# lucasjinreal/yolov7_d2

Hardware: AMD Instinct MI355X
Metric: images/sec training, YOLOX-s 640x640 bs=16/GPU (higher is better)
Workload: dtype bf16; 1 GPU; YOLOX-s CSPDarknet+PAFPN 640x640 bs=16/GPU: fwd + SimOTA loss + bwd + grad all-reduce + SGD(momentum) step, uint8 image batch + labels resident in HBM; global_batch=16, parallelism=dp1, hipgraph=True

## Files before the change

yolov7_d2_amd/csrc/conv3x3_ws.h:

```cpp
#pragma once
#include "common.h"
#include "conv_bn.h"

#define W3_MAX_JOBS 8
#define W3_TW 16
template <int S, int TH>
struct W3Geo {
  static constexpr int HH = S == 1 ? TH + 2 : 2 * TH + 1;
  static constexpr int HW = S == 1 ? W3_TW + 2 : 2 * W3_TW + 1;
  static constexpr int HPIX = HH * HW;
  static constexpr int HROWS = (HPIX + 63) / 64 * 64;
  static constexpr int tap(int dy, int dx) { return S == 1 ? dy * HW + dx : dy * HW + (dx & 1) * (W3_TW + 1) + (dx >> 1); }
};

struct W3Job {
  const __bf16* x;
  const u32x4* w;
  __bf16* y;
  double* stats;
  int ldx, ldy, N, H, W, tilesY, tilesX, ntiles;
  int blk0, nblk;
  int wld, nslots, sld, pad_;
  int tw[9];
  int inH;
  CBnFwd bn;
  int inW, xfw;
  const BnXf* xf;
};
struct W3K {
  int njobs, dbg;
  W3Job j[W3_MAX_JOBS];
};
struct W3Launch {
  int K, MODE, grid, lds, S, XF;
  W3K k;
};

#define W3_VMCNT(n) asm volatile("s_waitcnt vmcnt(%0)" ::"n"(n) : "memory")

static __device__ uint4 g_w3_zero_page[4];
static __device__ __attribute__((aligned(256))) unsigned g_w3_bar[MI_BN_BAR_WORDS];

__device__ __forceinline__ void w3_glds16(const void* g, unsigned lds_off) {
  asm volatile("s_mov_b32 m0, %1\n\ts_nop 0\n\tglobal_load_lds_dwordx4 %0, off" ::"v"(g), "s"(lds_off) : "memory");
}

template <int K, int WM, int WN, int G, int MODE, int S = 1, int TH = 8, int XF = 0>
__global__ __launch_bounds__(WM* WN * 64, (K == 128 || (S == 2 && K == 64)) ? 1 : 2) void w3_kernel(const W3K p) {
  static_assert(!XF || MODE == 1, "the input transform comes with the forward (statistics) mode");
  constexpr int NW = WM * WN, KC8 = K / 8, KS = K / 16;
  using Geo = W3Geo<S, TH>;
  constexpr int W3_TH = TH, W3_HW = Geo::HW, W3_HPIX = Geo::HPIX, W3_HROWS = Geo::HROWS;
  static_assert(WN * G * 32 == W3_TH * W3_TW, "pixel tile");
  constexpr int PLANE = W3_HROWS * 16;
  constexpr int NQ = (W3_HROWS / 64) * KC8;
  constexpr int D = NQ / NW;
  static_assert(NQ % NW == 0 && D >= 1, "DMA split");
  constexpr int XB = KC8 * PLANE;
  static_assert((KC8 - 1) * PLANE + Geo::tap(2, 2) * 16 < 65536, "ds_read immediate");
  constexpr int NS = 9 * KS, NTS = NS / 3;
  constexpr int NST = 2 * G;
  constexpr int DST = 2 * (D - 1) < NTS ? 2 : 1, SST = 2 * NST + NST / 2 <= NTS ? 2 : 1;
  static_assert(DST * (D - 1) < NTS && SST * NST + (MODE == 2 ? NST / 2 : 0) <= NTS, "the memory operations of a tile fit its main loop");

  extern __shared__ __attribute__((aligned(16))) char smem[];
  const unsigned lds0 = (unsigned)(uintptr_t)(__attribute__((address_space(3))) char*)smem;
  const int tid = threadIdx.x, lane = tid & 63;
  const int wave = __builtin_amdgcn_readfirstlane(tid >> 6);
  const int wm = wave / WN, wn = wave % WN;
  const int l31 = lane & 31, h = lane >> 5;

  int ji = 0;
  while (ji + 1 < p.njobs && (int)blockIdx.x >= p.j[ji + 1].blk0) ++ji;
  ji = __builtin_amdgcn_readfirstlane(ji);
  const W3Job& jb = p.j[ji];
  const int b = (int)blockIdx.x - jb.blk0, nb = jb.nblk;
  const int nt = (jb.ntiles - b + nb - 1) / nb;
  constexpr bool STATS = MODE == 1 || MODE == 3;
  unsigned gen0 = 0;
  if constexpr (MODE == 3) {
    const int nblk = (int)gridDim.x;
    if (tid == 0)
      gen0 = __hip_atomic_load(bn_bar_gen(g_w3_bar, (int)blockIdx.x % (nblk < BN_BAR_G ? nblk : BN_BAR_G)), __ATOMIC_RELAXED, __HIP_MEMORY_SCOPE_AGENT);
  }
  const int H = jb.H, Wd = jb.W, tilesX = jb.tilesX, tpi = jb.tilesY * jb.tilesX;
  const int inH = S == 1 ? jb.H : jb.inH, inW = S == 1 ? jb.W : jb.inW;
  const int ldxb = jb.ldx * 2, ldyb = jb.ldy * 2;
  const char* const xbase = (const char*)jb.x;
  char* const ybase = (char*)jb.y;
  const char* zpage = (const char*)g_w3_zero_page;
  asm volatile("" : "+s"(zpage));
  float* const s_sc = (float*)(smem + 2 * (K / 8) * Geo::HROWS * 16 + 256 * 32 * 4);
  float* const s_sh = s_sc + K;
  int xf_act = 0, xf_ldab = 0;
  char* xf_a = nullptr;
  if constexpr (XF) {
    const BnXf* const xf = jb.xf;
    bnx_tables(xf, s_sc, s_sh, NW * 64, jb.xfw != 0 && b == 0);
    xf_act = xf->bn.act;
    xf_ldab = xf->bn.lda * 2;
    xf_a = jb.xfw ? (char*)xf->bn.a : nullptr;
  }

  bf16x8 a[9][KS];
  {
    const u32x4* wb = jb.w + wm * 32 + l31;
#pragma unroll
    for (int t = 0; t < 9; ++t) {
      const int slab = jb.tw[t] * KC8;
#pragma unroll
      for (int ks = 0; ks < KS; ++ks) a[t][ks] = __builtin_bit_cast(bf16x8, wb[(size_t)(slab + ks * 2 + h) * jb.wld]);
    }
  }

  struct Org { int img, ty0, tx0; };
  auto tile_origin = [&](int i) {
    const int t = b + i * nb;
// ... 245 lines not shown
    }
  }
  if constexpr (MODE == 3) {
    int* const s_gave_up = (int*)(smem + 16384);
    bn_grid_barrier(g_w3_bar, gen0, (int)blockIdx.x, (int)gridDim.x, s_gave_up);
    const float poison = *s_gave_up ? __builtin_nanf("") : 0.f;
    const CBnFwd& bn = jb.bn;
    float scl, shl;
    cbn_finalize(bn, jb.stats + (wm * 32 + l31) * 2, jb.sld, jb.nslots, wm * 32 + l31, b == 0 && wn == 0 && h == 0, poison, scl, shl);
    float sc[2][8], sh[2][8];
#pragma unroll
    for (int pr = 0; pr < 2; ++pr)
#pragma unroll
      for (int e = 0; e < 8; ++e) {
        sc[pr][e] = __shfl(scl, pr * 16 + h * 8 + e, 64);
        sh[pr][e] = __shfl(shl, pr * 16 + h * 8 + e, 64);
      }
    const int act = bn.act;
    const bool has_res = bn.res != nullptr;
    const size_t ldab = (size_t)bn.lda * 2, ldrb = (size_t)bn.ldres * 2;
    char* const abase = (char*)bn.a + wm * 64 + h * 16;
    const char* const rbase = (const char*)bn.res + wm * 64 + h * 16;
    for (int i = 0; i < nt; ++i) {
      const Org o = tile_origin(i);
      u32x4 v[NST], r[NST];
      size_t pixi[G];
      bool ok[G];
#pragma unroll
      for (int g = 0; g < G; ++g) {
        const int py = o.ty0 + (wn * G + g) * 2 + lg, px = o.tx0 + lidx;
        ok[g] = (py < H) & (px < Wd);
        pixi[g] = ((size_t)o.img * H + py) * Wd + px;
#pragma unroll
        for (int pr = 0; pr < 2; ++pr) {
          v[g * 2 + pr] = r[g * 2 + pr] = u32x4{0u, 0u, 0u, 0u};
          if (ok[g]) {
            v[g * 2 + pr] = *(const u32x4*)(ybase + pixi[g] * (size_t)ldyb + wm * 64 + h * 16 + pr * 32);
            if (has_res) r[g * 2 + pr] = *(const u32x4*)(rbase + pixi[g] * ldrb + pr * 32);
          }
        }
      }
#pragma unroll
      for (int g = 0; g < G; ++g)
#pragma unroll
        for (int pr = 0; pr < 2; ++pr)
          if (ok[g]) *(u32x4*)(abase + pixi[g] * ldab + pr * 32) = cbn_apply8(v[g * 2 + pr], sc[pr], sh[pr], act, has_res, r[g * 2 + pr]);
    }
  }
}

template <int K, int WM, int WN, int G, int MODE, int S = 1, int TH = 8, int XF = 0>
static int w3_launch_one(const W3Launch& l, hipStream_t s) {
  auto fn = w3_kernel<K, WM, WN, G, MODE, S, TH, XF>;
  static bool attr_done = false;
  if (!attr_done) {
    hipFuncSetAttribute((const void*)fn, hipFuncAttributeMaxDynamicSharedMemorySize, 160 * 1024);
    attr_done = true;
  }
  hipLaunchKernelGGL(fn, dim3((unsigned)l.grid), dim3(WM * WN * 64), (size_t)l.lds, s, l.k);
  MI_CHECK_LAUNCH("conv3x3_ws");
  return MI_OK;
}
constexpr int w3_tile_h(int S, int K) { return S == 1 ? 8 : (K == 128 ? 2 : 4); }
constexpr int w3_block_cout(int S, int K) { return S == 1 ? K : (K == 32 ? 64 : 128); }
template <int MODE, int XF = 0>
static int w3_launch_mode(const W3Launch& l, hipStream_t s) {
  if (l.S == 2) {
    if constexpr (MODE == 1 || MODE == 0) {
      switch (l.K) {
        case 128: return w3_launch_one<128, 4, 1, 1, MODE, 2, 2, XF>(l, s);
        case 64: return w3_launch_one<64, 4, 1, 2, MODE, 2, 4, XF>(l, s);
        case 32: return w3_launch_one<32, 2, 2, 1, MODE, 2, 4, XF>(l, s);
      }
    }
    MI_FAIL(MI_EINVAL, "conv3x3_ws: stride 2 with K %d / mode %d", l.K, MODE);
  }
  switch (l.K) {
    case 128: return w3_launch_one<128, 4, 1, 4, MODE, 1, 8, XF>(l, s);
    case 64: return w3_launch_one<64, 2, 2, 2, MODE, 1, 8, XF>(l, s);
    case 32: return w3_launch_one<32, 1, 4, 1, MODE, 1, 8, XF>(l, s);
  }
  MI_FAIL(MI_EINVAL, "conv3x3_ws: K %d", l.K);
}
```

yolov7_d2_amd/csrc/conv3x3_ws.hip:

```cpp
#include <stdlib.h>
#include <string.h>
#include "common.h"
#include "conv3x3_ws.h"

int w3_launch_mode0(const W3Launch& l, hipStream_t s);
int w3_launch_mode1(const W3Launch& l, hipStream_t s);
int w3_launch_mode1x(const W3Launch& l, hipStream_t s);
int w3_launch_mode2(const W3Launch& l, hipStream_t s);
int w3_launch_mode3(const W3Launch& l, hipStream_t s);
int w3_mode3_blocks_per_cu(int K, int lds);
int w3_bar_status(unsigned* flag);
bool cbn_from_job(const mi_conv_desc& d, const mi_bn_job& j, CBnFwd* o);

static int w3_cus() {
  static int cus = 0;
  if (!cus) {
    int dev = 0;
    hipDeviceProp_t pr;
    if (hipGetDevice(&dev) == hipSuccess && hipGetDeviceProperties(&pr, dev) == hipSuccess) cus = pr.multiProcessorCount;
    if (cus <= 0) cus = 256;
  }
  return cus;
}

static bool w3_desc_ok(const mi_conv_desc* d, int* tw) {
  const int K = d->K8 * 8;
  if (d->ntaps != 9 || (d->in_stride != 1 && d->in_stride != 2) || d->out_stride != 1 || d->out_oy || d->out_ox) return false;
  if (d->gridH != d->outH || d->gridW != d->outW) return false;
  if (d->flags & ~MI_CONV_ACCUM) return false;
  if (d->bias) return false;
  if (!(K == 32 || K == 64 || K == 128) || d->Cout != d->CoutPad) return false;
  if (d->in_stride == 1) {
    if (d->outH != d->H || d->outW != d->W || d->Cout != K) return false;
  } else {
    const char* s2 = getenv("MI_CONV_WS_S2");
    if ((s2 && atoi(s2) == 0) || (d->flags & MI_CONV_ACCUM)) return false;
    if (d->outH != (d->H - 1) / 2 + 1 || d->outW != (d->W - 1) / 2 + 1) return false;
    const int bc = w3_block_cout(2, K);
    if (d->Cout % bc || d->Cout / bc > W3_MAX_JOBS) return false;
  }
  if (d->ldx % 8 || d->ldy % 8 || ((uintptr_t)d->x & 15) || ((uintptr_t)d->y & 15) || ((uintptr_t)d->w & 15)) return false;
  if (d->y_nstride && (long long)d->y_nstride != (long long)d->outH * d->outW * d->ldy) return false;
  if ((long long)d->H * d->W * d->ldx * 2 >= (1LL << 31)) return false;
  if ((d->flags & MI_CONV_ACCUM) && d->stats_acc) return false;
  int seen = 0;
  for (int t = 0; t < 9; ++t) {
    const int dy = d->tap_dy[t], dx = d->tap_dx[t];
    if (dy < -1 || dy > 1 || dx < -1 || dx > 1) return false;
    const int pos = (dy + 1) * 3 + dx + 1;
    if (seen & (1 << pos)) return false;
    seen |= 1 << pos;
    tw[pos] = d->tap_w[t];
  }
  return seen == 0x1ff;
}

static bool w3_fill(const mi_conv_desc* ds, int n, W3Launch* l, const mi_bn_job* bn = nullptr) {
  if (n < 1 || n > W3_MAX_JOBS) return false;
  memset(l, 0, sizeof(*l));
  const int K = ds[0].K8 * 8, S = ds[0].in_stride;
  if (bn && ((ds[0].flags & MI_CONV_ACCUM) || !ds[0].stats_acc || S != 1)) return false;
  const int mode = (ds[0].flags & MI_CONV_ACCUM) ? 2 : (ds[0].stats_acc ? (bn ? 3 : 1) : 0);
  const bool xf = ds[0].xf != nullptr;
  if (xf && mode != 1) return false;
  const int TH = w3_tile_h(S, K);
  const int hrows = ((S == 1 ? (TH + 2) * (W3_TW + 2) : (2 * TH + 1) * (2 * W3_TW + 1)) + 63) / 64 * 64;
  const int lds = 2 * (K / 8) * hrows * 16 + ((mode == 1 || mode == 3) ? 256 * 32 * 4 : 0) + (xf ? 2 * K * 4 : 0);
  long long total = 0;
  int nj = 0;
  for (int j = 0; j < n; ++j) {
    const mi_conv_desc& d = ds[j];
    int tw[9];
    if (!w3_desc_ok(&d, tw) || d.K8 * 8 != K || d.in_stride != S) return false;
    if ((d.flags & MI_CONV_ACCUM) != (ds[0].flags & MI_CONV_ACCUM) || (d.stats_acc != nullptr) != (ds[0].stats_acc != nullptr)) return false;
    if ((d.xf != nullptr) != xf || (xf && (d.xf_C != K || ((uintptr_t)d.xf & 7)))) return false;
    const int bc = w3_block_cout(S, K);
    for (int c0 = 0; c0 < d.Cout; c0 += bc, ++nj) {
      if (nj >= W3_MAX_JOBS) return false;
      W3Job& jb = l->k.j[nj];
      memcpy(jb.tw, tw, sizeof(tw));
      jb.x = (const __bf16*)d.x; jb.w = (const u32x4*)d.w + c0; jb.y = (__bf16*)d.y + c0;
      jb.stats = d.stats_acc ? d.stats_acc + (size_t)c0 * 2 : nullptr;
      jb.ldx = d.ldx; jb.ldy = d.ldy; jb.N = d.N; jb.H = d.outH; jb.W = d.outW; jb.inH = d.H; jb.inW = d.W;
      jb.tilesY = mi_cdiv(d.outH, TH); jb.tilesX = mi_cdiv(d.outW, W3_TW);
      jb.ntiles = d.N * jb.tilesY * jb.tilesX;
      jb.wld = d.CoutPad;
      jb.nslots = (d.stats_slots >= 1 && d.stats_slots <= MI_BN_SLOTS) ? d.stats_slots : MI_BN_SLOTS;
      jb.sld = d.CoutPad * 2;
      total += jb.ntiles;
      if (bn && !cbn_from_job(d, bn[j], &jb.bn)) return false;
      jb.xf = (const BnXf*)d.xf;
      jb.xfw = (xf && d.xf_write && c0 == 0) ? 1 : 0;
    }
  }
  n = nj;
  static const int ovr = getenv("MI_W3_PERCU") ? atoi(getenv("MI_W3_PERCU")) : 0;
  int per_cu = ovr > 0 ? ovr : (K == 128 ? 1 : (K == 64 ? 2 : 4));
  if (S == 2 && ovr <= 0) per_cu = (160 * 1024) / lds >= 2 && K != 128 ? 2 : 1;
  if (mode == 3) {
    static int occ[3] = {-1, -1, -1};
    int& o = occ[K == 128 ? 0 : (K == 64 ? 1 : 2)];
    if (o < 0) o = w3_mode3_blocks_per_cu(K, lds);
    if (o < 1) return false;
    if (per_cu > o) per_cu = o;
  }
  long long cap = (long long)w3_cus() * per_cu;
  if (cap > total) cap = total;
  int used = 0;
  for (int j = 0; j < n; ++j) {
    W3Job& jb = l->k.j[j];
    long long nb = (cap * jb.ntiles) / total;
    if (nb < 1) nb = 1;
    if (nb > jb.ntiles) nb = jb.ntiles;
    jb.nblk = (int)nb;
    used += jb.nblk;
  }
  while (used < cap) {
    int best = -1;
    double br = 0;
    for (int j = 0; j < n; ++j) {
      const W3Job& jb = l->k.j[j];
      const double r = (double)jb.ntiles / jb.nblk;
      if (jb.nblk < jb.ntiles && r > br) { br = r; best = j; }
    }
    if (best < 0) break;
    l->k.j[best].nblk++;
    used++;
  }
  int blk = 0;
  for (int j = 0; j < n; ++j) {
    l->k.j[j].blk0 = blk;
    blk += l->k.j[j].nblk;
  }
  l->k.njobs = n;
  l->k.dbg = (getenv("MI_DEBUG_NOATOM") ? atoi(getenv("MI_DEBUG_NOATOM")) & 1 : 0) | (getenv("MI_W3_DBG") ? atoi(getenv("MI_W3_DBG")) & 6 : 0);
  l->K = K;
  l->S = S;
  l->MODE = mode;
  l->XF = xf ? 1 : 0;
  l->grid = blk;
  l->lds = lds;
  return true;
}

static int w3_run(const W3Launch& l, hipStream_t s) {
  switch (l.MODE) {
    case 0: return w3_launch_mode0(l, s);
    case 1: return l.XF ? w3_launch_mode1x(l, s) : w3_launch_mode1(l, s);
    case 3: return w3_launch_mode3(l, s);
    default: return w3_launch_mode2(l, s);
  }
}

static bool w3_enabled() {
  const char* e = getenv("MI_CONV_WS");
  return !e || atoi(e) != 0;
}

bool w3_try_launch(const mi_conv_desc* ds, int n, hipStream_t s, int* rc) {
  if (!w3_enabled()) return false;
  W3Launch l;
  if (!w3_fill(ds, n, &l)) return false;
  *rc = w3_run(l, s);
  return true;
}
bool w3_try_plan(const mi_conv_desc* ds, int n, W3Launch* l) { return w3_enabled() && w3_fill(ds, n, l); }
bool w3_try_plan_bn(const mi_conv_desc* ds, const mi_bn_job* bn, int n, W3Launch* l) { return w3_enabled() && w3_fill(ds, n, l, bn); }
int w3_barrier_status(unsigned* flag) { return w3_bar_status(flag); }
int w3_run_planned(const W3Launch* l, hipStream_t s) { return w3_run(*l, s); }

extern "C" int mi_conv3x3_ws(const mi_conv_desc* descs, int n, mi_stream_t st) {
  MI_REQUIRE(descs && n >= 1, "conv3x3_ws: null");
  W3Launch l;
  MI_REQUIRE(w3_fill(descs, n, &l),
             "conv3x3_ws: needs 1..%d bf16 3x3 stride-1 convs with K == Cout in {32, 64, 128} (all the same K), no bias, "
             "all plain / all with stats_acc / all MI_CONV_ACCUM", W3_MAX_JOBS);
  return w3_run(l, (hipStream_t)st);
}
```

yolov7_d2_amd/csrc/conv_igemm.hip:

```cpp
#include <string.h>
#include <string.h>
#include "common.h"
#include "conv_igemm_kernel.h"
#include "conv1x1_stream.h"

bool c1s_try_launch(const mi_conv_desc* ds, int n, hipStream_t s, int* rc);
bool c1s_try_plan(const mi_conv_desc* ds, int n, C1Launch* l);
int c1s_run_planned(const C1Launch* l, hipStream_t s);
bool c1s_try_plan_bn(const mi_conv_desc* ds, const mi_bn_job* bn, int n, C1Launch* l);
int c1s_barrier_status(unsigned* flag);
static_assert(sizeof(C1Launch) <= sizeof(((mi_conv_group*)0)->priv), "mi_conv_group.priv holds the stream launch record");
#include "conv3x3_ws.h"
bool w3_try_launch(const mi_conv_desc* ds, int n, hipStream_t s, int* rc);
bool w3_try_plan(const mi_conv_desc* ds, int n, W3Launch* l);
int w3_run_planned(const W3Launch* l, hipStream_t s);
bool w3_try_plan_bn(const mi_conv_desc* ds, const mi_bn_job* bn, int n, W3Launch* l);
int w3_barrier_status(unsigned* flag);
static_assert(sizeof(W3Launch) <= sizeof(((mi_conv_group*)0)->priv), "mi_conv_group.priv holds the 3x3 launch record");

#define MI_DECL_KC(KCv)                                                                      \
  int conv_launch_kc##KCv(const ConvK& k, int BN, int TPIX, size_t lds, hipStream_t s);       \
  int conv_group_launch_kc##KCv(const mi_conv_group* m, const ConvK* jobs, const int* starts, hipStream_t s);
MI_DECL_KC(16) MI_DECL_KC(32) MI_DECL_KC(64) MI_DECL_KC(128)
#undef MI_DECL_KC

static void choose_tile(int TPIX, int gridH, int gridW, int* TH, int* TW) {
  const int cands[] = {gridW, 64, 32, 16, 8, 4};
  long best = -1;
  int bh = 8, bw = 16;
  for (int c : cands) {
    if (c <= 0 || c > TPIX) continue;
    int tw = c;
    int th = TPIX / tw;
    if (th > gridH) th = gridH;
    if (th < 1) th = 1;
    long tiles = (long)mi_cdiv(gridH, th) * mi_cdiv(gridW, tw);
    long halo = (long)(th + 2) * (tw + 2);
    long score = tiles * 100000 + halo;
    if (best < 0 || score < best) {
      best = score;
      bh = th;
      bw = tw;
    }
  }
  *TH = bh;
  *TW = bw;
}

struct ConvCfg {
  int KC, BN, TPIX, TPS;
};

#ifdef MI_CONV_TIMELINE
static long long* g_conv_tl = nullptr;
extern "C" void mi_debug_conv_timeline(long long* dev_buf) { g_conv_tl = dev_buf; }
#endif
static int conv_fill(const mi_conv_desc* d, ConvK* k, ConvCfg* c, size_t* ldsBytes) {
  MI_REQUIRE(d->x && d->w && d->y, "conv: null pointer");
  MI_REQUIRE(d->ntaps >= 1 && d->ntaps <= MI_MAX_TAPS, "conv: ntaps %d", d->ntaps);
  MI_REQUIRE(d->K8 >= 2 && (d->K8 % 2) == 0, "conv: K8 %d must be even", d->K8);
  MI_REQUIRE(d->CoutPad % 32 == 0 && d->Cout <= d->CoutPad && d->Cout > 0, "conv: Cout %d pad %d",
             d->Cout, d->CoutPad);
  MI_REQUIRE(d->ldx % 8 == 0 && ((uintptr_t)d->x % 16) == 0, "conv: x must be 16B aligned (ldx %d)", d->ldx);
  MI_REQUIRE(d->in_stride == 1 || d->in_stride == 2, "conv: in_stride");
  MI_REQUIRE(d->out_stride == 1 || d->out_stride == 2, "conv: out_stride");
  MI_REQUIRE((long long)d->H * d->W * d->ldx < (1LL << 30), "conv: image plane too large for 32-bit offsets");
  if (!(d->flags & MI_CONV_OUT_F32))
    MI_REQUIRE((d->Cout % 4 != 0) || (d->ldy % 4 == 0 && ((uintptr_t)d->y % 8) == 0),
               "conv: bf16 y needs 8B alignment (ldy %d)", d->ldy);
  k->x = (const __bf16*)d->x;
  k->w = (const u32x4*)d->w;
  k->y = d->y;
  k->bias = d->bias;
  k->stats = d->stats_acc;
  k->nslots = (d->stats_slots >= 1 && d->stats_slots <= MI_BN_SLOTS) ? d->stats_slots : MI_BN_SLOTS;
  k->ynstride = d->y_nstride > 0 ? (long long)d->y_nstride : (long long)d->outH * d->outW * d->ldy;
  k->ldx = d->ldx; k->ldy = d->ldy; k->N = d->N; k->H = d->H; k->W = d->W;
  k->outH = d->outH; k->outW = d->outW; k->gridH = d->gridH; k->gridW = d->gridW;
  k->is = d->in_stride; k->os = d->out_stride; k->ooy = d->out_oy; k->oox = d->out_ox;
  k->K8 = d->K8; k->Cout = d->Cout; k->CoutPad = d->CoutPad; k->ntaps = d->ntaps;
  int dymin = 1 << 30, dymax = -(1 << 30), dxmin = 1 << 30, dxmax = -(1 << 30);
  for (int t = 0; t < d->ntaps; ++t) {
    k->tw[t] = d->tap_w[t];
    if (d->tap_dy[t] < dymin) dymin = d->tap_dy[t];
    if (d->tap_dy[t] > dymax) dymax = d->tap_dy[t];
    if (d->tap_dx[t] < dxmin) dxmin = d->tap_dx[t];
    if (d->tap_dx[t] > dxmax) dxmax = d->tap_dx[t];
  }
  k->flags = d->flags;
  {
    static const int noatom = getenv("MI_DEBUG_NOATOM") ? atoi(getenv("MI_DEBUG_NOATOM")) : 0;
    if (noatom) k->flags |= 1024;
  }
  MI_REQUIRE(!(d->flags & MI_CONV_RELU) || !((d->flags & (MI_CONV_ACCUM | MI_CONV_BNBWD | MI_CONV_OUT_F32 | MI_CONV_RELUMASK | MI_CONV_ADDRELU)) || d->stats_acc),
             "conv: MI_CONV_RELU is a plain forward epilogue (bf16 output, no accumulate / statistics)");
  if (d->flags & MI_CONV_BNBWD) {
    MI_REQUIRE(d->stats_acc && d->bn_y && d->bn_scale && d->bn_shift && d->bn_mean && d->bn_invstd,
               "conv: MI_CONV_BNBWD needs stats_acc and the producing layer's bn_* arrays");
    MI_REQUIRE(!(d->flags & MI_CONV_OUT_F32) && d->Cout % 8 == 0 && d->bn_ldy % 8 == 0 && ((uintptr_t)d->bn_y % 16) == 0,
// ... 88 lines not shown
    }
    KC = bk; tps = bt;
  }
  MI_REQUIRE((KC == 16 || KC == 32 || KC == 64 || KC == 128) && Kp % KC == 0, "conv: KC %d for K %d", KC, Kp);
  MI_REQUIRE(tps >= 1 && d->ntaps % tps == 0, "conv: TPS %d for %d taps", tps, d->ntaps);
  const int RPI = 64 / (KC / 8);
  k->nqx = mi_cdiv(k->npixh, RPI);
  k->xbytes = k->nqx * 1024;
  MI_REQUIRE((long)k->nqx * RPI * k->haloW < (1 << 20) && k->nqx * RPI < 4096, "conv: halo too large for the row decode");
  k->mTW = ((1u << 20) + TW - 1) / TW;
  k->mHW = ((1u << 20) + k->haloW - 1) / k->haloW;
  const int nch = Kp / KC, nst = nch * (d->ntaps / tps);
  k->tps = tps;
  k->xstride = nch > 1 ? k->xbytes : 0;
  k->wstride = nst > 1 ? tps * (KC / 8) * BN * 16 : 0;
  c->KC = KC; c->BN = BN; c->TPIX = TPIX; c->TPS = tps;
  {
    static const int xm = getenv("MI_CONV_XMAP") ? atoi(getenv("MI_CONV_XMAP")) : 2;
    const bool on = xm >= 3 || (xm == 2 && (k->nco > 1 || d->ntaps > 1)) || (xm == 1 && k->nco > 1);
    k->xmap = (on && nblocks % 8 == 0) ? (int)(nblocks / 8) : 0;
#ifdef MI_CONV_TIMELINE
    k->tl = g_conv_tl;
#endif
  }
  *ldsBytes = lds_need(KC, tps);
  const size_t stage = (size_t)TPIX * (BN * 2 + 16);
  const size_t red = (size_t)16 * BN * 8;
  if (*ldsBytes < stage) *ldsBytes = stage;
  if (*ldsBytes < red) *ldsBytes = red;
  if (*ldsBytes < 4 * BN * 8) *ldsBytes = 4 * BN * 8;
  MI_REQUIRE(*ldsBytes <= 160 * 1024, "conv: LDS %zu too large", *ldsBytes);
  return MI_OK;
}

extern "C" int mi_conv2d_route(const mi_conv_desc* d) {
  MI_REQUIRE(d, "conv2d_route: null");
  C1Launch cl;
  if (c1s_try_plan(d, 1, &cl)) return 1;
  W3Launch wl;
  if (w3_try_plan(d, 1, &wl)) return 2;
  return d->xf ? -1 : 0;
}

extern "C" int mi_conv2d_plan(mi_conv_desc* d) {
  ConvK k;
  ConvCfg c;
  size_t lds;
  int rc = conv_fill(d, &k, &c, &lds);
  if (rc) return rc;
  d->TH = k.TH; d->TW = k.TW; d->KC = c.KC; d->BN = c.BN; d->TPS = c.TPS;
  return d->N * k.tilesY * k.tilesX;
}

extern "C" int mi_conv2d(const mi_conv_desc* d, mi_stream_t st) {
  {
    int rc = MI_OK;
    if (d && c1s_try_launch(d, 1, (hipStream_t)st, &rc)) return rc;
    if (d && w3_try_launch(d, 1, (hipStream_t)st, &rc)) return rc;
  }
  MI_REQUIRE(!d || !d->xf, "conv: the BatchNorm of the input (xf) runs on the streaming 1x1 / weight-stationary 3x3 kernels only");
  ConvK k;
  ConvCfg c;
  size_t lds;
  int rc = conv_fill(d, &k, &c, &lds);
  if (rc) return rc;
  hipStream_t s = (hipStream_t)st;
  static const long w8max = getenv("MI_CONV_W8") ? atol(getenv("MI_CONV_W8")) : (1L << 40);
  static const int w8mask = getenv("MI_CONV_W8MASK") ? atoi(getenv("MI_CONV_W8MASK")) : 7;
  const long nblocks = (long)k.N * k.tilesY * k.tilesX * k.nco;
  int tp = c.TPIX;
  const int cls = (c.TPIX == 128 && c.BN == 64) ? 1 : (c.TPIX == 128 && c.BN == 128) ? 2 : (c.TPIX == 64 && c.BN == 128) ? 4 : 0;
  if (nblocks <= w8max && (cls & w8mask) && !(d->flags & MI_CONV_OUT_F32) && (d->Cout & 7) == 0) {
    tp |= 1024;
  }
  switch (c.KC) {
    case 16: return conv_launch_kc16(k, c.BN, tp, lds, s);
    case 32: return conv_launch_kc32(k, c.BN, tp, lds, s);
    case 64: return conv_launch_kc64(k, c.BN, tp, lds, s);
    case 128: return conv_launch_kc128(k, c.BN, tp, lds, s);
  }
  MI_FAIL(MI_EINVAL, "conv: no kernel for KC %d BN %d TPIX %d", c.KC, c.BN, c.TPIX);
}

extern "C" int mi_conv2d_group_plan(const mi_conv_desc* descs, int n, void* table_host, int64_t table_cap,
                                    mi_conv_group* meta) {
  MI_REQUIRE(descs && meta && n >= 1 && n <= MI_CONV_MAX_GROUP, "conv_group_plan: 1..%d jobs", MI_CONV_MAX_GROUP);
  {
    C1Launch cl;
    if (c1s_try_plan(descs, n, &cl)) {
      memset(meta, 0, sizeof(*meta));
      meta->njobs = n; meta->nblocks = cl.grid; meta->lds_bytes = cl.lds;
      meta->KC = -1; meta->BN = cl.WM * 32; meta->TPIX = cl.PT; meta->TPS = cl.NBUF; meta->EPI = cl.MODE;
      meta->starts_off = 0; meta->table_bytes = 16;
      memcpy(meta->priv, &cl, sizeof(cl));
      if (table_host) {
        MI_REQUIRE(table_cap >= meta->table_bytes, "conv_group_plan: table too small");
        memset(table_host, 0, (size_t)meta->table_bytes);
      }
      return MI_OK;
    }
    W3Launch wl;
    if (w3_try_plan(descs, n, &wl)) {
      memset(meta, 0, sizeof(*meta));
      meta->njobs = n; meta->nblocks = wl.grid; meta->lds_bytes = wl.lds;
      meta->KC = -2; meta->BN = wl.K; meta->TPIX = 128; meta->TPS = 9; meta->EPI = wl.MODE;
      meta->starts_off = 0; meta->table_bytes = 16;
      memcpy(meta->priv, &wl, sizeof(wl));
      if (table_host) {
        MI_REQUIRE(table_cap >= meta->table_bytes, "conv_group_plan: table too small");
        memset(table_host, 0, (size_t)meta->table_bytes);
      }
      return MI_OK;
    }
  }
  for (int j = 0; j < n; ++j)
    MI_REQUIRE(!descs[j].xf, "conv_group_plan: the BatchNorm of the input (xf) runs on the streaming 1x1 / weight-stationary 3x3 kernels only");
  int big = 0;
  for (int j = 1; j < n; ++j)
    if ((long)descs[j].N * descs[j].gridH * descs[j].gridW > (long)descs[big].N * descs[big].gridH * descs[big].gridW) big = j;
  ConvK kb;
  ConvCfg cb;
  size_t lb;
  int rc = conv_fill(&descs[big], &kb, &cb, &lb);
  if (rc) return rc;
  ConvK ks[MI_CONV_MAX_GROUP];
  int starts[MI_CONV_MAX_GROUP + 1];
  size_t lds = 0;
  int epi = -1;
  starts[0] = 0;
  for (int j = 0; j < n; ++j) {
    mi_conv_desc d = descs[j];
    MI_REQUIRE((d.K8 * 8) % cb.KC == 0 && d.CoutPad % cb.BN == 0 && d.ntaps % cb.TPS == 0,
               "conv_group_plan: job %d does not fit the group's configuration (KC %d BN %d TPS %d)", j, cb.KC, cb.BN, cb.TPS);
    d.KC = cb.KC; d.BN = cb.BN; d.TPS = cb.TPS;
    ConvCfg c;
    size_t l = 0;
    if (j == big) {
      d.TH = kb.TH; d.TW = kb.TW;
      rc = conv_fill(&d, &ks[j], &c, &l);
      if (rc) return rc;
    } else {
      const size_t cap = lb > 80 * 1024 ? lb : 80 * 1024;
      const int cands[6][2] = {{0, 0}, {8, 16}, {4, 32}, {16, 8}, {8, 8}, {4, 16}};
      long bestTiles = -1;
      for (int q = 0; q < 6; ++q) {
        mi_conv_desc t = d;
        if (q == 0) {
          int th, tw;
          choose_tile(cb.TPIX, d.gridH, d.gridW, &th, &tw);
          t.TH = th; t.TW = tw;
        } else {
          t.TH = cands[q][0]; t.TW = cands[q][1];
        }
        if ((t.TH * t.TW <= 64 ? 64 : 128) != cb.TPIX) continue;
        ConvK kt;
        ConvCfg ct;
        size_t lt;
        if (conv_fill(&t, &kt, &ct, &lt) != MI_OK) continue;
        if (lt > cap || ct.KC != cb.KC || ct.BN != cb.BN || ct.TPS != cb.TPS) continue;
        const long tiles = (long)kt.N * kt.tilesY * kt.tilesX;
        if (bestTiles < 0 || tiles < bestTiles) { bestTiles = tiles; ks[j] = kt; c = ct; l = lt; }
      }
      MI_REQUIRE(bestTiles > 0, "conv_group_plan: job %d has no tile shape within the group's LDS footprint", j);
    }
    MI_REQUIRE(c.KC == cb.KC && c.BN == cb.BN && c.TPIX == cb.TPIX && c.TPS == cb.TPS,
               "conv_group_plan: job %d resolved to another configuration", j);
    MI_REQUIRE(!(ks[j].flags & (MI_CONV_RELUMASK | MI_CONV_ADDRELU)), "conv_group_plan: the aux-tensor epilogue (RELUMASK / ADDRELU) is a single-launch feature");
    const int e = (ks[j].flags & (MI_CONV_ACCUM | MI_CONV_BNBWD)) != 0;
    MI_REQUIRE(epi < 0 || epi == e, "conv_group_plan: jobs mix accumulating and plain launches");
    epi = e;
    if (l > lds) lds = l;
    if (starts[j] % 8) ks[j].xmap = 0;
    starts[j + 1] = starts[j] + ks[j].N * ks[j].tilesY * ks[j].tilesX * ks[j].nco;
  }
  int tpix = cb.TPIX;
  {
    static const long w8max = getenv("MI_CONV_W8G") ? atol(getenv("MI_CONV_W8G")) : (1L << 40);
    static const int w8mask = getenv("MI_CONV_W8MASK") ? atoi(getenv("MI_CONV_W8MASK")) : 7;
    const int cls = (cb.TPIX == 128 && cb.BN == 64) ? 1 : (cb.TPIX == 128 && cb.BN == 128) ? 2 : (cb.TPIX == 64 && cb.BN == 128) ? 4 : 0;
    bool staged = true;
    for (int j = 0; j < n; ++j) staged = staged && !(descs[j].flags & MI_CONV_OUT_F32) && (descs[j].Cout & 7) == 0;
    if (starts[n] <= w8max && (cls & w8mask) && staged) {
      tpix |= 1024;
    }
  }
  meta->njobs = n; meta->nblocks = starts[n]; meta->lds_bytes = (int32_t)lds;
  meta->KC = cb.KC; meta->BN = cb.BN; meta->TPIX = tpix; meta->TPS = cb.TPS; meta->EPI = epi;
  meta->starts_off = (int64_t)sizeof(ConvK) * n;
  meta->table_bytes = meta->starts_off + (int64_t)sizeof(int) * (n + 1);
  if (table_host) {
    MI_REQUIRE(table_cap >= meta->table_bytes, "conv_group_plan: table too small");
    memcpy(table_host, ks, sizeof(ConvK) * n);
    memcpy((char*)table_host + meta->starts_off, starts, sizeof(int) * (n + 1));
  }
  return MI_OK;
}

extern "C" int mi_conv2d_bn_plan(const mi_conv_desc* descs, const mi_bn_job* bn, int n, mi_conv_group* meta) {
  MI_REQUIRE(descs && bn && meta && n >= 1 && n <= MI_CONV_MAX_GROUP, "conv_bn_plan: 1..%d jobs", MI_CONV_MAX_GROUP);
  C1Launch cl;
  if (c1s_try_plan_bn(descs, bn, n, &cl)) {
    memset(meta, 0, sizeof(*meta));
    meta->njobs = n; meta->nblocks = cl.grid; meta->lds_bytes = cl.lds;
    meta->KC = -1; meta->BN = cl.WM * 32; meta->TPIX = cl.PT; meta->TPS = cl.NBUF; meta->EPI = cl.MODE;
    meta->table_bytes = 16;
    memcpy(meta->priv, &cl, sizeof(cl));
    return 1;
  }
  W3Launch wl;
  if (w3_try_plan_bn(descs, bn, n, &wl)) {
    memset(meta, 0, sizeof(*meta));
    meta->njobs = n; meta->nblocks = wl.grid; meta->lds_bytes = wl.lds;
    meta->KC = -2; meta->BN = wl.K; meta->TPIX = 128; meta->TPS = 9; meta->EPI = wl.MODE;
    meta->table_bytes = 16;
    memcpy(meta->priv, &wl, sizeof(wl));
    return 1;
  }
  return 0;
}

extern "C" int mi_conv2d_bn_fwd(const mi_conv_desc* descs, const mi_bn_job* bn, int n, mi_stream_t st) {
  mi_conv_group meta;
  const int rc = mi_conv2d_bn_plan(descs, bn, n, &meta);
  if (rc < 0) return rc;
  MI_REQUIRE(rc == 1, "conv_bn_fwd: needs convolutions that run on the streaming 1x1 (at most %d of one input) or the weight-"
             "stationary 3x3 kernel with stats_acc, each followed by the train-mode BatchNorm of exactly its output", C1_MAX_BN);
  if (meta.KC == -1) return c1s_run_planned((const C1Launch*)meta.priv, (hipStream_t)st);
  return w3_run_planned((const W3Launch*)meta.priv, (hipStream_t)st);
}

extern "C" int mi_conv_bn_barrier_status(uint32_t* flags) {
  MI_REQUIRE(flags, "conv_bn_barrier_status: null");
  unsigned a = 0, b = 0;
  int rc = c1s_barrier_status(&a);
  if (rc) return rc;
  rc = w3_barrier_status(&b);
  if (rc) return rc;
  *flags = (a ? 1u : 0u) | (b ? 2u : 0u);
  return MI_OK;
}

extern "C" int mi_conv2d_group_run(const mi_conv_group* m, const void* table_dev, mi_stream_t st) {
  MI_REQUIRE(m && (table_dev || m->KC < 0) && m->njobs >= 1, "conv_group_run: null");
  if (m->KC == -1) return c1s_run_planned((const C1Launch*)m->priv, (hipStream_t)st);
  if (m->KC == -2) return w3_run_planned((const W3Launch*)m->priv, (hipStream_t)st);
  const ConvK* jobs = (const ConvK*)table_dev;
  const int* starts = (const int*)((const char*)table_dev + m->starts_off);
  hipStream_t s = (hipStream_t)st;
  switch (m->KC) {
    case 16: return conv_group_launch_kc16(m, jobs, starts, s);
    case 32: return conv_group_launch_kc32(m, jobs, starts, s);
    case 64: return conv_group_launch_kc64(m, jobs, starts, s);
    case 128: return conv_group_launch_kc128(m, jobs, starts, s);
  }
  MI_FAIL(MI_EINVAL, "conv_group: no kernel for KC %d BN %d TPIX %d", m->KC, m->BN, m->TPIX);
}

__device__ __forceinline__ void pack_w_body(const float* __restrict__ w, int Cout, int Cin, int KK, __bf16* wf,
                                            int CinPad, int CoutPad, __bf16* wd, int CoutPadK, int CinPadN,
                                            const float* __restrict__ cs = nullptr) {
  const int64_t nf = wf ? (int64_t)KK * CinPad * CoutPad : 0;
  const int64_t nd = wd ? (int64_t)KK * CoutPadK * CinPadN : 0;
  for (int64_t idx = blockIdx.x * (int64_t)blockDim.x + threadIdx.x; idx < nf + nd;
       idx += (int64_t)gridDim.x * blockDim.x) {
    if (idx < nf) {
      const int e = idx & 7;
      int64_t r = idx >> 3;
      const int co = r % CoutPad; r /= CoutPad;
      const int k8 = r % (CinPad / 8);
      const int tap = r / (CinPad / 8);
      const int ci = k8 * 8 + e;
      float v = 0.f;
      if (co < Cout && ci < Cin) v = w[((int64_t)co * Cin + ci) * KK + tap] * (cs ? cs[co] : 1.f);
      wf[idx] = (__bf16)v;
    } else {
      const int64_t i2 = idx - nf;
      const int e = i2 & 7;
      int64_t r = i2 >> 3;
      const int ci = r % CinPadN; r /= CinPadN;
      const int k8 = r % (CoutPadK / 8);
      const int tap = r / (CoutPadK / 8);
      const int co = k8 * 8 + e;
      float v = 0.f;
      if (co < Cout && ci < Cin) v = w[((int64_t)co * Cin + ci) * KK + tap] * (cs ? cs[co] : 1.f);
      wd[i2] = (__bf16)v;
    }
  }
}

__global__ void pack_w_kernel(const float* __restrict__ w, int Cout, int Cin, int KK, __bf16* wf, int CinPad,
                              int CoutPad, __bf16* wd, int CoutPadK, int CinPadN) {
  pack_w_body(w, Cout, Cin, KK, wf, CinPad, CoutPad, wd, CoutPadK, CinPadN);
}
__global__ void pack_w_scaled_kernel(const float* __restrict__ w, const float* __restrict__ cs, int Cout, int Cin, int KK,
                                     __bf16* wf, int CinPad, int CoutPad, __bf16* wd, int CoutPadK, int CinPadN) {
  pack_w_body(w, Cout, Cin, KK, wf, CinPad, CoutPad, wd, CoutPadK, CinPadN, cs);
}
#define PK_CO 32
#define PK_CI 64
__global__ __launch_bounds__(256) void pack_w_batch_kernel(const mi_pack_job* __restrict__ jobs, int njobs, int kk_max) {
  extern __shared__ __attribute__((aligned(16))) __bf16 pk_s[];
  int lo = 0, hi = njobs - 1;
  while (lo < hi) {
    const int mid = (lo + hi + 1) >> 1;
    if (jobs[mid].blk0 <= (int)blockIdx.x) lo = mid; else hi = mid - 1;
  }
  const mi_pack_job j = jobs[lo];
  const int KK = j.KK, tid = threadIdx.x;
  const int coP = j.wd && j.CoutPadK > j.CoutPad ? j.CoutPadK : (j.wf ? j.CoutPad : j.CoutPadK);
  const int nco_t = (coP + PK_CO - 1) / PK_CO;
  const int t = (int)blockIdx.x - j.blk0;
  const int co0 = (t % nco_t) * PK_CO, ci0 = (t / nco_t) * PK_CI;
  const int rs = PK_CI * kk_max + 2;
  int nci = j.Cin - ci0;
  nci = nci < 0 ? 0 : (nci > PK_CI ? PK_CI : nci);
  const int rowlen = PK_CI * KK;
  const float* const wrow0 = j.w + ((size_t)co0 * j.Cin + ci0) * KK;
  const bool fast = nci == PK_CI && co0 + PK_CO <= j.Cout && ((j.Cin * KK) & 3) == 0 && (((uintptr_t)wrow0) & 15) == 0 &&
                    (rowlen & 3) == 0;
  if (fast) {
    const int wave = tid >> 6, lane = tid & 63;
    for (int co_l = wave; co_l < PK_CO; co_l += 4) {
      const float4* src = (const float4*)(wrow0 + (size_t)co_l * j.Cin * KK);
      const float sc = j.scale ? j.scale[co0 + co_l] : 1.f;
      unsigned* dst = (unsigned*)(pk_s + co_l * rs);
      for (int q4 = lane; q4 < rowlen / 4; q4 += 64) {
        const float4 v = src[q4];
        const __bf16 b0 = (__bf16)(v.x * sc), b1 = (__bf16)(v.y * sc), b2 = (__bf16)(v.z * sc), b3 = (__bf16)(v.w * sc);
// ... 107 lines not shown
```

Measured before the change: 3080 images/sec.

## Add weight-stationary kernel for stride-2 3x3 conv data gradient

Measured after the change: 3110 images/sec (median of 6 runs). Within noise of the previous version (+1.0%).

```diff
diff --git a/yolov7_d2_amd/csrc/conv3x3_ws.h b/yolov7_d2_amd/csrc/conv3x3_ws.h
--- a/yolov7_d2_amd/csrc/conv3x3_ws.h
+++ b/yolov7_d2_amd/csrc/conv3x3_ws.h
@@ -26,6 +26,7 @@
   CBnFwd bn;
   int inW, xfw;
   const BnXf* xf;
+  int oH, oW;
 };
 struct W3K {
   int njobs, dbg;
@@ -33,6 +34,7 @@
 };
 struct W3Launch {
   int K, MODE, grid, lds, S, XF;
+  int D2, WM;
   W3K k;
 };
 
@@ -444,3 +446,182 @@
   }
   MI_FAIL(MI_EINVAL, "conv3x3_ws: K %d", l.K);
 }
+
+__host__ __device__ constexpr int w3d_cls(int q) { return q < 1 ? 0 : q < 3 ? 1 : q < 5 ? 2 : 3; }
+__host__ __device__ constexpr int w3d_oy(int q) { return (q == 3 || q == 5 || q == 6) ? 1 : 0; }
+__host__ __device__ constexpr int w3d_ox(int q) { return (q == 1 || q == 5 || q == 7) ? 1 : 0; }
+__host__ __device__ constexpr int w3d_first(int c) { return c == 0 ? 0 : c == 1 ? 1 : c == 2 ? 3 : 5; }
+__host__ __device__ constexpr int w3d_ntaps(int c) { return c == 0 ? 1 : c == 3 ? 4 : 2; }
+
+template <int K, int WM, int WN>
+__global__ __launch_bounds__(WM* WN * 64, K == 128 ? 1 : 2) void w3d_kernel(const W3K p) {
+  constexpr int G = 1, NW = WM * WN, KC8 = K / 8, KS = K / 16, TH = WN * G * 2;
+  using Geo = W3Geo<1, TH>;
+  constexpr int W3_HW = Geo::HW, W3_HPIX = Geo::HPIX, W3_HROWS = Geo::HROWS;
+  constexpr int PLANE = W3_HROWS * 16;
+  constexpr int NQ = (W3_HROWS / 64) * KC8, D = NQ / NW;
+  static_assert(NQ % NW == 0 && D >= 1 && D <= 4 * KS, "DMA split: one instruction per k-step of the last class");
+  constexpr int XB = KC8 * PLANE;
+  static_assert((KC8 - 1) * PLANE + Geo::tap(2, 2) * 16 < 65536, "ds_read immediate");
+  constexpr int NS = 9 * KS, NST = 2 * G;
+
+  extern __shared__ __attribute__((aligned(16))) char smem[];
+  const unsigned lds0 = (unsigned)(uintptr_t)(__attribute__((address_space(3))) char*)smem;
+  const int tid = threadIdx.x, lane = tid & 63;
+  const int wave = __builtin_amdgcn_readfirstlane(tid >> 6);
+  const int wm = wave / WN, wn = wave % WN;
+  const int l31 = lane & 31, h = lane >> 5;
+
+  const W3Job& jb = p.j[0];
+  const int b = (int)blockIdx.x, nb = jb.nblk;
+  const int nt = (jb.ntiles - b + nb - 1) / nb;
+  const int H = jb.H, Wd = jb.W, tilesX = jb.tilesX, tpi = jb.tilesY * jb.tilesX;
+  const int oH = jb.oH, oW = jb.oW;
+  const int ldxb = jb.ldx * 2, ldyb = jb.ldy * 2;
+  const char* const xbase = (const char*)jb.x;
+  char* const ybase = (char*)jb.y;
+  const char* zpage = (const char*)g_w3_zero_page;
+  asm volatile("" : "+s"(zpage));
+
+  bf16x8 a[9][KS];
+  {
+    const u32x4* wb = jb.w + wm * 32 + l31;
+#pragma unroll
+    for (int q = 0; q < 9; ++q) {
+      const int slab = jb.tw[q] * KC8;
+#pragma unroll
+      for (int ks = 0; ks < KS; ++ks) a[q][ks] = __builtin_bit_cast(bf16x8, wb[(size_t)(slab + ks * 2 + h) * jb.wld]);
+    }
+  }
+
+  struct Org { int img, ty0, tx0; };
+  auto tile_origin = [&](int i) {
+    const int t = b + i * nb;
+    Org o;
+    o.img = t / tpi;
+    const int rem = t - o.img * tpi, tyq = rem / tilesX;
+    o.ty0 = tyq * TH;
+    o.tx0 = (rem - tyq * tilesX) * W3_TW;
+    return o;
+  };
+  auto issue_x1 = [&](const Org& o, int buf, int d) {
+    const int iy0 = o.ty0 - 1, ix0 = o.tx0 - 1;
+    const char* xt = xbase + ((size_t)o.img * H * Wd + (ptrdiff_t)iy0 * Wd + ix0) * (ptrdiff_t)ldxb;
+    const int q = wave * D + d;
+    const int pb = q / KC8, k8 = q % KC8;
+    const int pix = pb * 64 + lane;
+    const int hy = (int)(((unsigned)pix * 3641u) >> 16);
+    const int hx = pix - hy * W3_HW;
+    const bool v = (pix < W3_HPIX) & ((unsigned)(iy0 + hy) < (unsigned)H) & ((unsigned)(ix0 + hx) < (unsigned)Wd);
+    const char* g = v ? xt + (unsigned)((hy * Wd + hx) * ldxb + k8 * 16) : zpage;
+    w3_glds16(g, lds0 + buf * XB + k8 * PLANE + pb * 1024);
+  };
+
+  int lg, lidx;
+  {
+    const int l = l31;
+    lg = ((l >= 4) & (l < 12)) | ((l >= 16) & (l < 20)) | (l >= 28);
+    lidx = l - (l < 4 ? 0 : l < 12 ? 4 : l < 20 ? 8 : l < 28 ? 12 : 16);
+  }
+  const unsigned bbase = (unsigned)(h * PLANE + ((wn * G) * 2 + lg) * W3_HW * 16 + lidx * 16);
+  auto out_ptr = [&](const Org& o, int c) -> char* {
+    const int py = 2 * (o.ty0 + wn * G * 2 + lg) + (c >> 1), px = 2 * (o.tx0 + lidx) + (c & 1);
+    char* q = ybase + (((size_t)o.img * oH + py) * oW + px) * (size_t)ldyb + wm * 64 + h * 16;
+    return ((py < oH) & (px < oW)) ? q : nullptr;
+  };
+
+  Org oc = tile_origin(0), op = oc;
+#pragma unroll
+  for (int d = 0; d < D; ++d) issue_x1(oc, 0, d);
+
+  u32x4 pk[NST];
+#pragma unroll
+  for (int q = 0; q < NST; ++q) pk[q] = u32x4{0u, 0u, 0u, 0u};
+  for (int i = 0; i < nt; ++i) {
+    W3_VMCNT(0);
+    __builtin_amdgcn_s_barrier();
+    const bool more = i + 1 < nt;
+    const Org on = tile_origin(more ? i + 1 : i);
+    const char* Xs = smem + (i & 1) * XB;
+    f32x16 acc;
+    auto ldb = [&](int step, bf16x8& dst) {
+      const int q = step / KS, ks = step % KS;
+      dst = __builtin_bit_cast(bf16x8, *(const u32x4*)(Xs + bbase + (2 * ks * PLANE + Geo::tap(w3d_oy(q) + 1, w3d_ox(q) + 1) * 16)));
+    };
+    bf16x8 bf[3];
+    ldb(0, bf[0]);
+    ldb(1, bf[1]);
+#pragma unroll
+    for (int q = 0; q < 9; ++q)
+#pragma unroll
+    for (int ks = 0; ks < KS; ++ks) {
+      const int c = w3d_cls(q), st = q * KS + ks;
+      const int s0 = w3d_first(c) * KS, s1 = (w3d_first(c) + w3d_ntaps(c)) * KS;
+      __builtin_amdgcn_sched_barrier(0);
+      if (st == s0) {
+        {
+          const Org& po = c == 0 ? op : oc;
+          char* const pq = (c > 0 || i > 0) ? out_ptr(po, (c + 3) & 3) : nullptr;
+          if (pq) {
+#pragma unroll
+            for (int l = 0; l < NST; ++l) *(u32x4*)(pq + (l % 2) * 32) = pk[l];
+          }
+        }
+#pragma unroll
+        for (int r = 0; r < 16; ++r) acc[r] = 0.f;
+      }
+      if (c == 3 && st - s0 < D) {
+        if (more) issue_x1(on, (i + 1) & 1, st - s0);
+      }
+      if (st + 2 < NS) ldb(st + 2, bf[(st + 2) % 3]);
+      acc = __builtin_amdgcn_mfma_f32_32x32x16_bf16(a[q][ks], bf[st % 3], acc, 0, 0, 0);
+      __builtin_amdgcn_sched_group_barrier(0x008, 1, 0);
+      __builtin_amdgcn_sched_group_barrier(0x100, 1, 0);
+      __builtin_amdgcn_sched_group_barrier(0x002, 2, 0);
+      if (st == s1 - 1) {
+        __builtin_amdgcn_sched_barrier(0);
+        unsigned pw[8];
+#pragma unroll
+        for (int qq = 0; qq < 4; ++qq) {
+          bf16x4 o;
+#pragma unroll
+          for (int e = 0; e < 4; ++e) o[e] = (__bf16)acc[4 * qq + e];
+          const u32x2 u = __builtin_bit_cast(u32x2, o);
+          pw[2 * qq] = u[0];
+          pw[2 * qq + 1] = u[1];
+        }
+#pragma unroll
+        for (int pr = 0; pr < 2; ++pr) {
+          const int q0 = 2 * pr, q1 = 2 * pr + 1;
+          const auto w0 = __builtin_amdgcn_permlane32_swap(pw[2 * q0], pw[2 * q1], false, false);
+          const auto w1 = __builtin_amdgcn_permlane32_swap(pw[2 * q0 + 1], pw[2 * q1 + 1], false, false);
+          pk[pr] = u32x4{w0[0], w1[0], w0[1], w1[1]};
+        }
+      }
+    }
+    __builtin_amdgcn_sched_barrier(0);
+    op = oc;
+    oc = on;
+  }
+  if (nt > 0) {
+    char* const pq = out_ptr(op, 3);
+    if (pq) {
+#pragma unroll
+      for (int l = 0; l < NST; ++l) *(u32x4*)(pq + (l % 2) * 32) = pk[l];
+    }
+  }
+}
+
+template <int K, int WM>
+static int w3d_launch_one(const W3Launch& l, hipStream_t s) {
+  auto fn = w3d_kernel<K, WM, 4 / WM>;
+  static bool attr_done = false;
+  if (!attr_done) {
+    hipFuncSetAttribute((const void*)fn, hipFuncAttributeMaxDynamicSharedMemorySize, 160 * 1024);
+    attr_done = true;
+  }
+  hipLaunchKernelGGL(fn, dim3((unsigned)l.grid), dim3(256), (size_t)l.lds, s, l.k);
+  MI_CHECK_LAUNCH("conv3x3_ws (stride-2 data gradient)");
+  return MI_OK;
+}
+constexpr int w3d_tile_h(int WM) { return 2 * (4 / WM); }
diff --git a/yolov7_d2_amd/csrc/conv3x3_ws.hip b/yolov7_d2_amd/csrc/conv3x3_ws.hip
--- a/yolov7_d2_amd/csrc/conv3x3_ws.hip
+++ b/yolov7_d2_amd/csrc/conv3x3_ws.hip
@@ -8,6 +8,7 @@
 int w3_launch_mode1x(const W3Launch& l, hipStream_t s);
 int w3_launch_mode2(const W3Launch& l, hipStream_t s);
 int w3_launch_mode3(const W3Launch& l, hipStream_t s);
+int w3d_launch(const W3Launch& l, hipStream_t s);
 int w3_mode3_blocks_per_cu(int K, int lds);
 int w3_bar_status(unsigned* flag);
 bool cbn_from_job(const mi_conv_desc& d, const mi_bn_job& j, CBnFwd* o);
@@ -143,7 +144,62 @@
   return true;
 }
 
+static bool w3_fill_s2d(const mi_conv_desc* ds, int n, int KC, W3Launch* l) {
+  if (n != 4) return false;
+  const mi_conv_desc& d0 = ds[0];
+  const int K = d0.K8 * 8, C = d0.Cout;
+  if (!(K == 64 || K == 128) || KC != K || !(C == 32 || C == 64 || C == 128) || d0.CoutPad != C) return false;
+  if (d0.H != (d0.outH + 1) / 2 || d0.W != (d0.outW + 1) / 2) return false;
+  if (d0.ldx < K || d0.ldx % 8 || d0.ldy % 8 || ((uintptr_t)d0.x & 15) || ((uintptr_t)d0.y & 15) || ((uintptr_t)d0.w & 15)) return false;
+  if (d0.y_nstride && (long long)d0.y_nstride != (long long)d0.outH * d0.outW * d0.ldy) return false;
+  if ((long long)d0.H * d0.W * d0.ldx * 2 >= (1LL << 31)) return false;
+  memset(l, 0, sizeof(*l));
+  W3Job& jb = l->k.j[0];
+  int seen = 0;
+  for (int j = 0; j < n; ++j) {
+    const mi_conv_desc& d = ds[j];
+    if (d.x != d0.x || d.w != d0.w || d.y != d0.y || d.ldx != d0.ldx || d.ldy != d0.ldy || d.y_nstride != d0.y_nstride ||
+        d.N != d0.N || d.H != d0.H || d.W != d0.W || d.outH != d0.outH || d.outW != d0.outW || d.K8 != d0.K8 ||
+        d.Cout != C || d.CoutPad != C || d.flags != d0.flags)
+      return false;
+    if (d.flags || d.bias || d.stats_acc || d.xf) return false;
+    if (d.in_stride != 1 || d.out_stride != 2 || (d.out_oy & ~1) || (d.out_ox & ~1)) return false;
+    const int c = d.out_oy * 2 + d.out_ox;
+    if (seen & (1 << c)) return false;
+    seen |= 1 << c;
+    if (d.gridH != (d.outH - d.out_oy + 1) / 2 || d.gridW != (d.outW - d.out_ox + 1) / 2) return false;
+    if (d.ntaps != w3d_ntaps(c)) return false;
+    for (int t = 0; t < d.ntaps; ++t) {
+      const int q = w3d_first(c) + t;
+      if (d.tap_dy[t] != w3d_oy(q) || d.tap_dx[t] != w3d_ox(q) || d.tap_w[t] < 0 || d.tap_w[t] >= 9) return false;
+      jb.tw[q] = d.tap_w[t];
+    }
+  }
+  if (seen != 15) return false;
+  const int WM = C / 32, TH = w3d_tile_h(WM);
+  jb.x = (const __bf16*)d0.x; jb.w = (const u32x4*)d0.w; jb.y = (__bf16*)d0.y;
+  jb.ldx = d0.ldx; jb.ldy = d0.ldy; jb.N = d0.N; jb.H = jb.inH = d0.H; jb.W = jb.inW = d0.W;
+  jb.oH = d0.outH; jb.oW = d0.outW;
+  jb.tilesY = mi_cdiv(d0.H, TH); jb.tilesX = mi_cdiv(d0.W, W3_TW);
+  jb.ntiles = d0.N * jb.tilesY * jb.tilesX;
+  jb.wld = d0.CoutPad;
+  long long cap = (long long)w3_cus() * (K == 128 ? 1 : 2);
+  if (cap > jb.ntiles) cap = jb.ntiles;
+  jb.nblk = (int)cap;
+  jb.blk0 = 0;
+  l->k.njobs = 1;
+  l->K = K;
+  l->S = 2;
+  l->MODE = 0;
+  l->D2 = 1;
+  l->WM = WM;
+  l->grid = jb.nblk;
+  l->lds = 2 * (K / 8) * (((TH + 2) * (W3_TW + 2) + 63) / 64 * 64) * 16;
+  return true;
+}
+
 static int w3_run(const W3Launch& l, hipStream_t s) {
+  if (l.D2) return w3d_launch(l, s);
   switch (l.MODE) {
     case 0: return w3_launch_mode0(l, s);
     case 1: return l.XF ? w3_launch_mode1x(l, s) : w3_launch_mode1(l, s);
@@ -165,6 +221,11 @@
   return true;
 }
 bool w3_try_plan(const mi_conv_desc* ds, int n, W3Launch* l) { return w3_enabled() && w3_fill(ds, n, l); }
+bool w3_s2d_enabled() {
+  const char* e = getenv("MI_W3_S2_DGRAD");
+  return w3_enabled() && !(e && atoi(e) == 0);
+}
+bool w3_try_plan_s2d(const mi_conv_desc* ds, int n, int KC, W3Launch* l) { return w3_s2d_enabled() && w3_fill_s2d(ds, n, KC, l); }
 bool w3_try_plan_bn(const mi_conv_desc* ds, const mi_bn_job* bn, int n, W3Launch* l) { return w3_enabled() && w3_fill(ds, n, l, bn); }
 int w3_barrier_status(unsigned* flag) { return w3_bar_status(flag); }
 int w3_run_planned(const W3Launch* l, hipStream_t s) { return w3_run(*l, s); }
diff --git a/yolov7_d2_amd/csrc/conv3x3_ws_d2.hip b/yolov7_d2_amd/csrc/conv3x3_ws_d2.hip
--- /dev/null
+++ b/yolov7_d2_amd/csrc/conv3x3_ws_d2.hip
@@ -0,0 +1,9 @@
+#include "conv3x3_ws.h"
+int w3d_launch(const W3Launch& l, hipStream_t s) {
+  const int wm = l.WM;
+  switch (l.K) {
+    case 128: return wm == 4 ? w3d_launch_one<128, 4>(l, s) : wm == 2 ? w3d_launch_one<128, 2>(l, s) : w3d_launch_one<128, 1>(l, s);
+    case 64: return wm == 4 ? w3d_launch_one<64, 4>(l, s) : wm == 2 ? w3d_launch_one<64, 2>(l, s) : w3d_launch_one<64, 1>(l, s);
+  }
+  MI_FAIL(MI_EINVAL, "conv3x3_ws: stride-2 data gradient with K %d", l.K);
+}
diff --git a/yolov7_d2_amd/csrc/conv_igemm.hip b/yolov7_d2_amd/csrc/conv_igemm.hip
--- a/yolov7_d2_amd/csrc/conv_igemm.hip
+++ b/yolov7_d2_amd/csrc/conv_igemm.hip
@@ -15,6 +15,8 @@
 bool w3_try_plan(const mi_conv_desc* ds, int n, W3Launch* l);
 int w3_run_planned(const W3Launch* l, hipStream_t s);
 bool w3_try_plan_bn(const mi_conv_desc* ds, const mi_bn_job* bn, int n, W3Launch* l);
+bool w3_s2d_enabled();
+bool w3_try_plan_s2d(const mi_conv_desc* ds, int n, int KC, W3Launch* l);
 int w3_barrier_status(unsigned* flag);
 static_assert(sizeof(W3Launch) <= sizeof(((mi_conv_group*)0)->priv), "mi_conv_group.priv holds the 3x3 launch record");
 
@@ -269,6 +271,8 @@
   MI_FAIL(MI_EINVAL, "conv: no kernel for KC %d BN %d TPIX %d", c.KC, c.BN, c.TPIX);
 }
 
+static int conv_group_plan_tile(const mi_conv_desc* descs, int n, void* table_host, int64_t table_cap, mi_conv_group* meta);
+
 extern "C" int mi_conv2d_group_plan(const mi_conv_desc* descs, int n, void* table_host, int64_t table_cap,
                                     mi_conv_group* meta) {
   MI_REQUIRE(descs && meta && n >= 1 && n <= MI_CONV_MAX_GROUP, "conv_group_plan: 1..%d jobs", MI_CONV_MAX_GROUP);
@@ -300,6 +304,28 @@
       return MI_OK;
     }
   }
+  if (n == 4 && w3_s2d_enabled()) {
+    mi_conv_group tm;
+    const int rc = conv_group_plan_tile(descs, n, nullptr, 0, &tm);
+    if (rc) return rc;
+    W3Launch wl;
+    if (w3_try_plan_s2d(descs, n, tm.KC, &wl)) {
+      memset(meta, 0, sizeof(*meta));
+      meta->njobs = n; meta->nblocks = wl.grid; meta->lds_bytes = wl.lds;
+      meta->KC = -3; meta->BN = wl.WM * 32; meta->TPIX = 128; meta->TPS = 9; meta->EPI = wl.MODE;
+      meta->starts_off = 0; meta->table_bytes = 16;
+      memcpy(meta->priv, &wl, sizeof(wl));
+      if (table_host) {
+        MI_REQUIRE(table_cap >= meta->table_bytes, "conv_group_plan: table too small");
+        memset(table_host, 0, (size_t)meta->table_bytes);
+      }
+      return MI_OK;
+    }
+  }
+  return conv_group_plan_tile(descs, n, table_host, table_cap, meta);
+}
+
+static int conv_group_plan_tile(const mi_conv_desc* descs, int n, void* table_host, int64_t table_cap, mi_conv_group* meta) {
   for (int j = 0; j < n; ++j)
     MI_REQUIRE(!descs[j].xf, "conv_group_plan: the BatchNorm of the input (xf) runs on the streaming 1x1 / weight-stationary 3x3 kernels only");
   int big = 0;
@@ -430,7 +456,7 @@
 extern "C" int mi_conv2d_group_run(const mi_conv_group* m, const void* table_dev, mi_stream_t st) {
   MI_REQUIRE(m && (table_dev || m->KC < 0) && m->njobs >= 1, "conv_group_run: null");
   if (m->KC == -1) return c1s_run_planned((const C1Launch*)m->priv, (hipStream_t)st);
-  if (m->KC == -2) return w3_run_planned((const W3Launch*)m->priv, (hipStream_t)st);
+  if (m->KC == -2 || m->KC == -3) return w3_run_planned((const W3Launch*)m->priv, (hipStream_t)st);
   const ConvK* jobs = (const ConvK*)table_dev;
   const int* starts = (const int*)((const char*)table_dev + m->starts_off);
   hipStream_t s = (hipStream_t)st;
```
